# fudan-zvg/NeRF-LiDAR

Hardware: AMD Instinct MI355X
Metric: LiDAR rays/sec @128 samples/ray, 8x256 MLP; depth L1 vs reference (higher is better)
Workload: dtype f32 (sampling, hash grid) + split-bf16 x3 MFMA (density/semantic/intensity) + bf16 MFMA (view MLP); 1 GPU; C2: nuScenes 32-beam sweep, 32x1024 rays per sweep, samples (64,64,128), 8x256 NerfMLP + semantic + intensity heads, full-size fp32 hash tables; azimuth_columns_total=1024, parallelism=azimuth-sector x1, hip_graph_replay=False, weights=seeded synthetic (white-noise tables, x1500 density gain), sweep_origins=moving: step i renders sweep i mod 64 (pre-uploaded ray batches), gather_bytes_per_ray=1347584

## Files before the change

include/nerflidar_hip.h:

```cpp
#ifndef NERFLIDAR_HIP_H
#define NERFLIDAR_HIP_H

#include <stddef.h>
#include <stdint.h>

#ifdef __cplusplus
extern "C" {
#endif

#define NLR_MAX_LEVELS 4
#define NLR_MAX_GRID_LEVELS 16
#define NLR_MAX_VIEW_DEPTH 16

enum {
    NLR_OK = 0,
    NLR_ERR_INVALID = -1,
    NLR_ERR_UNSUPPORTED = -2,
    NLR_ERR_HIP = -3,
    NLR_ERR_WORKSPACE = -4
};

enum {
    NLR_PREC_F32 = 0,
    NLR_PREC_MIXED = 1,
// ... 60 lines not shown
    NlrLinear sem0, sem2;
    uint32_t use_intensity;
    NlrLinear int0, int2;
    float density_bias, rgb_premultiplier, rgb_bias, rgb_padding;
    uint32_t re_weights;
} NlrMlpDesc;

typedef struct NlrModelDesc {
    uint32_t num_levels;
    uint32_t num_samples[NLR_MAX_LEVELS];
    const NlrMlpDesc *mlps[NLR_MAX_LEVELS];
    float dilation_multiplier, dilation_bias;
    float anneal_slope, resample_padding;
    float power_lambda, std_scale;
    float bg_intensity;
    uint32_t opaque_background;
    uint32_t mlp_precision;
} NlrModelDesc;

typedef struct NlrModel NlrModel;
int nlr_model_create(const NlrModelDesc *desc, NlrModel **out, void *stream);
void nlr_model_destroy(NlrModel *m);
int nlr_model_set_table(NlrModel *m, uint32_t level, const void *table_dev, int table_dtype);

typedef struct NlrRays {
    const float *origins, *directions, *viewdirs;
    const float *radii, *near, *far;
    const float *base_x, *base_y;
} NlrRays;

typedef struct NlrRenderCfg {
    float train_frac;
    uint32_t compute_extras;
    uint32_t sample_n, sample_m;
    const float *rand_jitter[NLR_MAX_LEVELS];
    const float *rand_deg[NLR_MAX_LEVELS];
    float scale_factor;
    uint32_t shuffled_rays;
} NlrRenderCfg;

typedef struct NlrLevelOut {
    float *sdist, *tdist;
    float *weights, *density;
    float *rgb;
    float *semantic;
    float *intensity;
// ... 22 lines not shown
                     const NlrOut *out, void *workspace, size_t workspace_bytes, void *stream);

const char *nlr_kernel_names(void);

const char *nlr_build_sha(void);

#define NLR_DBG_FORCE_GENERIC 0
#define NLR_DBG_MLP_WORKGROUPS 1
#define NLR_DBG_BINNED_C4 2
#define NLR_DBG_NO_XPAIR_SCATTER 3
#define NLR_DBG_SCATTER_LEVELS 4
#define NLR_DBG_NO_SCATTER_CACHE 5
#define NLR_DBG_RAY_GROUPS 6
#define NLR_DBG_LAST_ROUTE 7
#define NLR_DBG_TRAIN_ROUTE 8
#define NLR_DBG_TRAIN_TRUNK_ROW0 9
#define NLR_DBG_TRAIN_TRUNK_ROWS 10
int nlr_debug_set(uint32_t key, int value);
int nlr_debug_get(uint32_t key);
int nlr_grid_fast_path(const int32_t *offsets_host, uint32_t L, uint32_t C, float S, uint32_t H, int table_dtype, uint32_t gridtype,
                       int align_corners, uint32_t interp);
int nlr_grid_level_plan(const int32_t *offsets_host, uint32_t L, uint32_t C, float S, uint32_t H, uint32_t gridtype, int align_corners,
                        uint32_t B, uint32_t *mode, uint32_t *step, uint32_t *lds_kind);

enum { NLR_K_RESAMPLE = 0, NLR_K_PROP = 1, NLR_K_ENCODE = 2, NLR_K_DIRBIAS = 3, NLR_K_MLP = 4, NLR_K_COMPOSITE = 5, NLR_K_COUNT = 6 };
int nlr_profile_begin(NlrModel *m);
int nlr_profile_begin_kinds(NlrModel *m, uint32_t kind_mask);
int nlr_profile_end(NlrModel *m, void *stream, float *total_ms, uint32_t *launches);

int nlr_resample_level(const float *prev_sdist, const float *prev_weights, uint32_t n_prev,
                       float dilation, float anneal, float resample_padding, uint32_t num_samples,
                       const float *rand_jitter, const float *near, const float *far,
                       float power_lambda, uint32_t N, float *sdist, float *tdist, void *stream);

int nlr_mlp_level(const NlrModel *m, uint32_t level, const NlrRays *rays, const float *tdist,
                  uint32_t N, uint32_t sample_n, uint32_t sample_m, const float *rand_deg,
                  float *features , float *density, float *rgb,
                  float *semantic, float *intensity, void *workspace, size_t workspace_bytes,
                  void *stream);

int nlr_composite_level(const float *density, const float *tdist, const float *directions,
                        const float *rgb, const float *semantic, const float *intensity,
                        const float *far, const float *origins, uint32_t N, uint32_t S,
                        uint32_t class_num, int opaque_background, float bg, int compute_extras,
                        float scale_factor, float *weights, const NlrOut *out, float *level_depth,
                        void *stream);
// ... 139 lines not shown
```

nerf-lidar_amd/csrc/nlr_api.hip:

```cpp
#include <stdarg.h>

#include <vector>

#include "nlr_kernels.h"

#include <stdlib.h>
#include "nlr_objects.h"
#include "nlr_tape.h"


static thread_local char g_err[512] = "";
void nlr_set_error(const char *fmt, ...) {
    va_list ap;
    va_start(ap, fmt);
    vsnprintf(g_err, sizeof(g_err), fmt, ap);
    va_end(ap);
}
extern "C" const char *nlr_last_error(void) { return g_err; }
extern "C" int nlr_version(void) { return 100; }
extern "C" const char *nlr_kernel_names(void) {
    return "nlr_resample_kernel,nlr_prop8_kernel,nlr_encode8_kernel,nlr_direnc_kernel,nlr_mlp_kernel,nlr_composite_kernel";
}

struct Profile {
// ... 21 lines not shown

struct MlpShape {
    uint32_t W = 0, WB = 0, D = 0, HT = 0, K = 0, int_row = 0xffffffffu, deg = 0, E = 0;
    bool use_int = false;
    uint32_t prec = NLR_PREC_MIXED;
    float rgb_premul = 1.0f, rgb_bias = 0.0f, rgb_padding = 0.001f;
};
struct LevelModel : MlpShape {
    bool is_prop = false;
    GridParams gp;
    uint32_t F = 0, S = 0;
    int re_weights = 1;
    float density_bias = -1.0f;
    float *p_w1 = nullptr, *p_b1 = nullptr, *p_w2 = nullptr;
    float p_b2 = 0.0f;
    void *tape = nullptr;
    uint32_t tape_chunks = 0;
    void *tape_lidar = nullptr;
    uint32_t tape_lidar_chunks = 0;
    float *bias_all = nullptr;
    uint32_t bias_count = 0;
    float *u_det = nullptr, *u_rand = nullptr;
    float max_jitter = 0.0f;
};

struct NlrModel {
    uint32_t num_levels = 0;
    LevelModel lv[NLR_MAX_LEVELS];
    float dilation_multiplier, dilation_bias, anneal_slope, resample_padding, power_lambda, std_scale, bg;
    uint32_t opaque, prec;
    int device = 0;
    uint32_t cus = 0;
    hipStream_t up = nullptr;
    std::vector<void *> allocs;
    mutable Profile prof;
};

static int dev_upload(NlrModel *m, const void *host, size_t bytes, void **out) {
    void *p = nullptr;
    NLR_HIP(hipMalloc(&p, bytes ? bytes : 16));
    m->allocs.push_back(p);
    if (bytes) {
        NLR_HIP(hipMemcpyAsync(p, host, bytes, hipMemcpyHostToDevice, m->up));
        NLR_HIP(hipStreamSynchronize(m->up));
    }
    *out = p;
// ... 283 lines not shown
                nlr_set_error("single_mlp / NerfMLP as proposal network has no fused path (level %u)", l);
                rc = NLR_ERR_UNSUPPORTED;
            }
        }
        if (rc) {
            nlr_model_destroy(m);
            return rc;
        }
    }
    if (hipStreamSynchronize(m->up) != hipSuccess) {
        nlr_model_destroy(m);
        NLR_FAIL(NLR_ERR_HIP, "model_create: weight upload failed");
    }
    *out = m;
    return NLR_OK;
}

extern "C" void nlr_model_destroy(NlrModel *m) {
    if (!m) return;
    for (void *p : m->allocs) (void)hipFree(p);
    delete m;
}

extern "C" int nlr_model_set_table(NlrModel *m, uint32_t level, const void *table_dev, int table_dtype) {
    NLR_CHECK_ARG(m && level < m->num_levels && table_dev, "model_set_table: bad argument");
    NLR_CHECK_ARG(table_dtype == 0 || table_dtype == 1, "model_set_table: table_dtype must be 0 or 1");
    m->lv[level].gp.table = table_dev;
    m->lv[level].gp.table_dtype = table_dtype;
    return NLR_OK;
}

extern "C" int nlr_profile_begin_kinds(NlrModel *m, uint32_t kind_mask) {
    NLR_CHECK_ARG(m != nullptr, "profile_begin: NULL model");
    for (hipEvent_t e : m->prof.ev) (void)hipEventDestroy(e);
    m->prof.ev.clear();
    m->prof.kind.clear();
    m->prof.mask = kind_mask;
    m->prof.armed = true;
    return NLR_OK;
}
extern "C" int nlr_profile_begin(NlrModel *m) { return nlr_profile_begin_kinds(m, 0xffffffffu); }

extern "C" int nlr_profile_end(NlrModel *m, void *stream, float *total_ms, uint32_t *launches) {
    NLR_CHECK_ARG(m && total_ms && launches, "profile_end: NULL argument");
    m->prof.armed = false;
    NLR_HIP(hipStreamSynchronize((hipStream_t)stream));
    for (int k = 0; k < NLR_K_COUNT; ++k) {
        total_ms[k] = 0.0f;
        launches[k] = 0;
    }
    for (size_t i = 0; i < m->prof.kind.size(); ++i) {
// ... 297 lines not shown
```

nerf-lidar_amd/csrc/nlr_common.h:

```cpp
#pragma once
#include <hip/hip_runtime.h>
#include <math.h>
#include <stdint.h>
#include <stdio.h>
#include <string.h>

#include "../../include/nerflidar_hip.h"
#include "nlr_tape.h"

#define NLR_EPS 1.1920928955078125e-07f
#define NLR_WAVE 64

void nlr_set_error(const char *fmt, ...);
#define NLR_FAIL(code, ...)         \
    do {                            \
        nlr_set_error(__VA_ARGS__); \
        return (code);              \
    } while (0)
#define NLR_CHECK_ARG(cond, ...) \
    do {                         \
        if (!(cond)) NLR_FAIL(NLR_ERR_INVALID, __VA_ARGS__); \
    } while (0)
#define NLR_HIP(call)                                                                      \
    do {                                                                                   \
// ... 7 lines not shown
        if (e_ != hipSuccess)                                                              \
            NLR_FAIL(NLR_ERR_HIP, "launch of %s failed: %s", name, hipGetErrorString(e_)); \
    } while (0)
static inline int nlr_tape_check(const char *what, size_t built, size_t program) {
    char msg[256];
    if (!nlr_tape_matches(what, built, program, msg, sizeof(msg))) NLR_FAIL(NLR_ERR_UNSUPPORTED, "%s", msg);
    return NLR_OK;
}

struct GridParams {
    const void *table;
    int32_t table_dtype;
    uint32_t L, C;
    uint32_t gridtype, align_corners, interp;
    uint32_t offset[NLR_MAX_GRID_LEVELS];
    uint32_t hsize[NLR_MAX_GRID_LEVELS];
    uint32_t res[NLR_MAX_GRID_LEVELS];
    float scale[NLR_MAX_GRID_LEVELS];
    float gsize[NLR_MAX_GRID_LEVELS];
    float inv_gsize[NLR_MAX_GRID_LEVELS];
    uint32_t dense[NLR_MAX_GRID_LEVELS];
    uint32_t mode[NLR_MAX_GRID_LEVELS];
    uint32_t step[NLR_MAX_GRID_LEVELS];
};

int nlr_fill_grid_params(GridParams *gp, const void *table, int table_dtype, const int32_t *offsets_host,
                         uint32_t L, uint32_t C, float S, uint32_t H, uint32_t gridtype, int align_corners,
                         uint32_t interp);

#ifdef __HIPCC__
__device__ __forceinline__ uint32_t nlr_grid_index(uint32_t gridtype, uint32_t align_corners, uint32_t hsize,
                                                   uint32_t res, uint32_t x, uint32_t y, uint32_t z) {
    uint32_t stride = 1, index = 0;
    const uint32_t step = align_corners ? res : res + 1;
    if (stride <= hsize) { index += x * stride; stride *= step; }
    if (stride <= hsize) { index += y * stride; stride *= step; }
    if (stride <= hsize) { index += z * stride; stride *= step; }
    if (gridtype == 0 && stride > hsize) index = x ^ (y * 2654435761u) ^ (z * 805459861u);
    return index % hsize;
}

template <int MODE>
__device__ __forceinline__ void nlr_corner_idx(const GridParams &gp, uint32_t level, const uint32_t (&pg)[3], uint32_t (&idx)[8]) {
    if (MODE == 0) {
        const uint32_t s = gp.step[level];
        const uint32_t y0 = pg[1] * s, z0 = pg[2] * s * s;
        const uint32_t y1 = y0 + s, z1 = z0 + s * s;
// ... 49 lines not shown
```

nerf-lidar_amd/csrc/nlr_encode.hip:

```cpp
#include "nlr_kernels.h"

#include <stdlib.h>

#include "nlr_cast.h"
#include "nlr_grid_level.h"
#include "nlr_level_fast.h"

template <typename T, int C>
__global__ void __launch_bounds__(256) nlr_encode_kernel(CastParams cp, GridParams gp, int re_weights, float *__restrict__ feat) {
    const uint32_t m = blockIdx.x * blockDim.x + threadIdx.x;
    const uint32_t M = cp.N * cp.S;
    if (m >= M) return;
    const uint32_t level = blockIdx.y;
    const uint32_t ray = m / cp.S, k = m - ray * cp.S;
    const RayRegs rr = nlr_load_ray(cp, ray, k);
    const float gsize = gp.gsize[level];
    float acc[C];
#pragma unroll
    for (int c = 0; c < C; ++c) acc[c] = 0.0f;
    for (uint32_t j = 0; j < cp.n; ++j) {
        const Gauss g = nlr_cast_one(cp, ray, k, j, rr);
        const float werf = re_weights ? nlr_erf_weight(g.zs, gsize) : 1.0f;
        nlr_level_accum<T, C>(gp, level, g, werf, acc);
    }
// ... 258 lines not shown
                for (int c = 0; c < 4; ++c) f0[c] = a[c] * inv_n, f1[c] = a[4 + c] * inv_n;
                continue;
            }
            float *f = nlr_feat_ptr<C>(feat, piece_major, M, m, l, gp.L);
            if constexpr (C == 4) {
                const nlr_f4 q = {a[0] * inv_n, a[1] * inv_n, a[2] * inv_n, a[3] * inv_n};
                __builtin_nontemporal_store(q, (nlr_f4 *)f);
            } else {
#pragma unroll
                for (int c = 0; c < C; ++c) f[c] = a[c] * inv_n;
            }
        }
    }
}

template <typename T, int C>
__global__ void __launch_bounds__(256) nlr_encode8_kernel(CastParams cp, GridParams gp, int re_weights, float *__restrict__ feat,
                                                          int piece_major, uint32_t nblocks, uint32_t chunk) {
    for (uint32_t b = blockIdx.x; b < nblocks; b += gridDim.x)
        nlr_encode8_block<T, C>(cp, gp, re_weights, feat, piece_major, chunk ? nlr_xcd_block(b, nblocks, chunk) : b);
}

template <typename T, int C, int LMAX>
__global__ void __launch_bounds__(256) nlr_prop8_kernel(CastParams cp, GridParams gp, PropMlpParams mp, int re_weights,
                                                        float *__restrict__ density, float *__restrict__ feat_out, uint32_t nblocks, uint32_t chunk) {
    __shared__ float sw[64 * 16 + 128];
    for (uint32_t i = threadIdx.x; i < 64 * mp.F; i += 256) sw[i] = mp.w1[i];
    if (threadIdx.x < 64) {
        sw[64 * mp.F + threadIdx.x] = mp.b1[threadIdx.x];
        sw[64 * mp.F + 64 + threadIdx.x] = mp.w2[threadIdx.x];
    }
    __syncthreads();
  for (uint32_t lb = blockIdx.x; lb < nblocks; lb += gridDim.x) {
    const uint32_t gt = (chunk ? nlr_xcd_block(lb, nblocks, chunk) : lb) * 256u + threadIdx.x;
    const uint32_t j = gt & 7;
    uint32_t pray, k;
    const bool in = nlr_slot_sample(cp, gt >> 3, pray, k);
    const uint32_t ray = NLR_DBG_RAY(pray);
    const uint32_t m = ray * cp.S + k;
    const bool active = in && j < cp.n;
    const RayRegs rr = nlr_load_ray(cp, ray, k);
    const Gauss g = nlr_cast_one(cp, ray, k, active ? j : 0, rr);
    const bool valid = active && !((g.x0 < 0 || g.x0 > 1) || (g.x1 < 0 || g.x1 > 1) || (g.x2 < 0 || g.x2 > 1));
    const float inv_s8 = __frsqrt_rn(8.0f * (g.zs * g.zs));
    const float inv_n = 1.0f / (float)cp.n;
    float feat[LMAX * C];
#pragma unroll
    for (int i = 0; i < LMAX * C; ++i) feat[i] = 0.0f;
    if (valid) {
#pragma unroll
        for (int l = 0; l < LMAX; ++l) {
            if (l < (int)gp.L) {
                const float werf = re_weights ? nlr_erf_weight_fast(inv_s8, gp.inv_gsize[l]) : 1.0f;
                float a[C];
                if (gp.mode[l] == 0) nlr_level_fast<T, C, 0>(gp, l, g.x0, g.x1, g.x2, werf, a);
                else nlr_level_fast<T, C, 1>(gp, l, g.x0, g.x1, g.x2, werf, a);
#pragma unroll
                for (int c = 0; c < C; ++c) feat[l * C + c] = a[c];
            }
        }
    }
    static_assert((LMAX * C) % 4 == 0, "feature count of the proposal kernel must be a multiple of 4");
#pragma unroll
    for (int i = 0; i < LMAX * C; i += 4) {
        float q[4] = {feat[i], feat[i + 1], feat[i + 2], feat[i + 3]};
        nlr_group8_sum_n(q);
#pragma unroll
        for (int u = 0; u < 4; ++u) feat[i + u] = q[u] * inv_n;
    }
    if (feat_out && in && j == 0)
        for (uint32_t i = 0; i < mp.F; ++i) feat_out[(size_t)m * mp.F + i] = feat[i];
    float part = 0.0f;
#pragma unroll
    for (int hh = 0; hh < 8; ++hh) {
        const uint32_t hu = hh * 8 + j;
        float a = sw[64 * mp.F + hu];
#pragma unroll
        for (int i = 0; i < LMAX * C; ++i)
            if (i < (int)mp.F) a = fmaf(sw[hu * mp.F + i], feat[i], a);
// ... 257 lines not shown
```

nerf-lidar_amd/csrc/nlr_grid.hip:

```cpp
#include "nlr_common.h"
#include "nlr_grid_level.h"

#include <hip/hip_fp16.h>

void nlr_level_scale(uint32_t L, float S, uint32_t H, float *scale, uint32_t *resolution) {
    for (uint32_t l = 0; l < L; ++l) {
        float sc = exp2f((float)l * S) * (float)H - 1.0f;
        scale[l] = sc;
        resolution[l] = (uint32_t)ceilf(sc) + 1u;
    }
}

int nlr_fill_grid_params(GridParams *gp, const void *table, int table_dtype, const int32_t *offsets_host,
                         uint32_t L, uint32_t C, float S, uint32_t H, uint32_t gridtype, int align_corners,
                         uint32_t interp) {
    NLR_CHECK_ARG(L >= 1 && L <= NLR_MAX_GRID_LEVELS, "grid: num_levels %u outside [1,%d]", L, NLR_MAX_GRID_LEVELS);
    NLR_CHECK_ARG(C == 1 || C == 2 || C == 4 || C == 8, "GridEncoding: C must be 1, 2, 4, or 8 (got %u)", C);
    NLR_CHECK_ARG(table_dtype == 0 || table_dtype == 1, "grid: table_dtype must be 0 (f32) or 1 (f16)");
    NLR_CHECK_ARG(offsets_host != nullptr, "grid: offsets (host) is NULL");
    memset(gp, 0, sizeof(*gp));
    gp->table = table;
    gp->table_dtype = table_dtype;
    gp->L = L;
    gp->C = C;
// ... 4 lines not shown
    for (uint32_t l = 0; l < L; ++l) {
        NLR_CHECK_ARG(offsets_host[l + 1] > offsets_host[l], "grid: offsets must be increasing (level %u)", l);
        gp->offset[l] = (uint32_t)offsets_host[l];
        gp->hsize[l] = (uint32_t)(offsets_host[l + 1] - offsets_host[l]);
        double r = ceil((double)H * exp2((double)l * (double)S));
        gp->gsize[l] = (float)((int)r + (align_corners ? 0 : 1));
        gp->inv_gsize[l] = 1.0f / gp->gsize[l];
        uint64_t step = align_corners ? gp->res[l] : gp->res[l] + 1, stride = 1;
        int dense = 1;
        for (int d = 0; d < 3; ++d) {
            if (stride > gp->hsize[l]) break;
            stride *= step;
        }
        if (gridtype == 0 && stride > gp->hsize[l]) dense = 0;
        gp->dense[l] = dense;
        gp->step[l] = (uint32_t)step;
        const uint32_t hs = gp->hsize[l];
        const bool all3 = (step <= hs) && (step * step <= hs);
        const bool walk = all3 && step * step * step <= hs;
        const uint64_t cmax = (uint64_t)floorf(fmaf(1.0f, gp->scale[l], align_corners ? 0.0f : 0.5f)) + 1u;
        if (walk && cmax * (1 + step + step * step) < hs) gp->mode[l] = 0;
        else if (!walk && gridtype == 0 && (hs & (hs - 1)) == 0) gp->mode[l] = 1;
        else gp->mode[l] = 2;
    }
    return NLR_OK;
}

template <typename T>
__device__ __forceinline__ float ld(const T *p);
template <>
__device__ __forceinline__ float ld<float>(const float *p) { return *p; }
template <>
__device__ __forceinline__ float ld<__half>(const __half *p) { return __half2float(*p); }

template <typename T, int C, bool DYDX>
__global__ void __launch_bounds__(256) nlr_grid_fwd_kernel(const float *__restrict__ x, GridParams gp, float *__restrict__ out,
                                                           float *__restrict__ dy_dx, uint32_t B, int out_layout) {
    const uint32_t b = blockIdx.x * blockDim.x + threadIdx.x;
    if (b >= B) return;
    const uint32_t level = blockIdx.y;
    const uint32_t L = gp.L;
    const T *grid = (const T *)gp.table + (size_t)gp.offset[level] * C;
    float *o = out_layout == 0 ? out + ((size_t)level * B + b) * C : out + (size_t)b * L * C + level * C;
    float *dd = DYDX ? dy_dx + (size_t)b * 3 * L * C + (size_t)level * 3 * C : nullptr;

    const float x0 = x[(size_t)b * 3 + 0], x1 = x[(size_t)b * 3 + 1], x2 = x[(size_t)b * 3 + 2];
// ... 711 lines not shown
```

nerf-lidar_amd/csrc/nlr_kernels.h:

```cpp
#pragma once
#include "nlr_common.h"

#define NLR_MAX_MULTI 16

struct CastParams {
    const float *origins, *directions, *base_x, *base_y, *radii;
    const float *tdist;
    const float *rand_deg;
    uint32_t N, S, n;
    uint32_t ray_groups, vote_min;
    const uint32_t *votes;
    float std_scale;
    float cosd[NLR_MAX_MULTI], sind[NLR_MAX_MULTI];
    float degj[NLR_MAX_MULTI];
};

struct PropMlpParams {
    const float *w1, *b1;
    const float *w2;
    float b2, density_bias;
    uint32_t F;
};

struct CompositeParams {
// ... 39 lines not shown
    uint32_t lidar;
};

struct DirEncParams {
    const float *viewdirs;
    const float *dirs;
    uint32_t N, deg, E;
    float *out;
    float *dnorm;
};
int nlr_launch_dnorm(const float *dirs, uint32_t N, float *dnorm, hipStream_t st);

int nlr_launch_resample(const float *prev_sdist, const float *prev_weights, uint32_t n_prev, float dilation, float anneal,
                        float pad, uint32_t S, const float *u_dev, const float *jitter, float max_jitter, const float *near,
                        const float *far, float lam, uint32_t N, float *sdist, float *tdist, hipStream_t st);
int nlr_fill_cast_params(CastParams *cp, const NlrRays *rays, const float *tdist, const float *rand_deg, uint32_t N,
                         uint32_t S, uint32_t n, uint32_t mloops, float std_scale);
int nlr_encode_features_args(CastParams *cp, GridParams *gp, const NlrRays *rays, const float *tdist, uint32_t N, uint32_t S, uint32_t sample_n,
                             uint32_t sample_m, float std_scale, const float *rand_deg, const NlrGridDesc *grid);
int nlr_launch_encode(const CastParams &cp, const GridParams &gp, int re_weights, float *feat, int piece_major, hipStream_t st);
int nlr_launch_ray_vote(const float *tdist, uint32_t N, uint32_t S, uint32_t *votes, hipStream_t st);
int nlr_launch_prop(const CastParams &cp, const GridParams &gp, const float *w1, const float *b1, const float *w2, float b2,
                    float density_bias, int re_weights, float *density, float *feat_out, hipStream_t st);
int nlr_launch_direnc(const DirEncParams &P, hipStream_t st);
int nlr_launch_mlp(const MlpParams &P, uint32_t W, uint32_t WB, uint32_t HT, uint32_t prec, uint32_t cus, hipStream_t st);
bool nlr_mlp_can_composite(uint32_t W, uint32_t WB, uint32_t HT, uint32_t prec, uint32_t F, uint32_t S, uint32_t K, bool use_int, uint64_t M,
                           uint32_t mode = 1);
int nlr_launch_composite(const CompositeParams &P, hipStream_t st);
int nlr_composite_segments(const float *density, const float *tdist, const float *directions, const float *seg, uint32_t class_num,
                           int has_intensity, const float *far, const float *origins, uint32_t N, uint32_t S, int opaque_background,
                           float bg, int compute_extras, float scale_factor, float *weights, const NlrOut *out, float *level_depth,
                           hipStream_t st, bool no_rgb = false);
int nlr_composite_level_impl(const float *density, const float *tdist, const float *directions, const float *rgb, const float *semantic,
                             const float *intensity, const float *far, const float *origins, uint32_t N, uint32_t S, uint32_t class_num,
                             int opaque_background, float bg, int compute_extras, float scale_factor, float *weights, const NlrOut *out,
                             float *level_depth, hipStream_t st, bool no_rgb);
```

nerf-lidar_amd/csrc/nlr_level_fast.h:

```cpp
#pragma once
#include "nlr_grid_level.h"

typedef float nlr_f2 __attribute__((ext_vector_type(2)));
#ifdef NLR_DBG_ENV
__device__ int nlr_dbg[8] = {0, 99, 0, 0, 0, 0, 0, 0};
#endif

template <typename T, int C>
struct NlrEntry;
template <>
struct NlrEntry<float, 1> {
    static constexpr int E = 2;
    static __device__ __forceinline__ void ld(const char *base, uint32_t off, float (&v)[1]) { v[0] = *(const float *)(base + off); }
};
template <>
struct NlrEntry<float, 2> {
    static constexpr int E = 3;
    static __device__ __forceinline__ void ld(const char *base, uint32_t off, float (&v)[2]) {
        const float2 t = *(const float2 *)(base + off);
        v[0] = t.x, v[1] = t.y;
    }
};
typedef float nlr_f4 __attribute__((ext_vector_type(4)));
template <>
// ... 100 lines not shown
template <>
struct NlrPair<__half, 4> {
    static constexpr bool ok = true;
    static __device__ __forceinline__ void ld(const char *base, uint32_t off, float (&a)[4], float (&b)[4]) {
        const nlr_uint4_a8 t = *(const nlr_uint4_a8 *)(base + off);
        const uint32_t w[4] = {t.x, t.y, t.z, t.w};
#pragma unroll
        for (int i = 0; i < 2; ++i) {
            const __half2 p = __builtin_bit_cast(__half2, w[i]), q = __builtin_bit_cast(__half2, w[2 + i]);
            a[2 * i] = __low2float(p), a[2 * i + 1] = __high2float(p), b[2 * i] = __low2float(q), b[2 * i + 1] = __high2float(q);
        }
    }
};

static inline bool nlr_level_fast_ok(const GridParams &gp) {
    if (gp.interp != 0 || gp.align_corners != 0) return false;
    const uint64_t entry = (uint64_t)gp.C * (gp.table_dtype == 0 ? 4 : 2);
    for (uint32_t l = 0; l < gp.L; ++l) {
        if (gp.mode[l] > 1) return false;
        if ((uint64_t)gp.hsize[l] * entry > (1ull << 32)) return false;
        if (gp.res[l] >= (1u << 30)) return false;
    }
    return true;
}

typedef uint32_t nlr_u2 __attribute__((ext_vector_type(2)));
typedef uint32_t nlr_u4 __attribute__((ext_vector_type(4)));
typedef uint32_t nlr_u8 __attribute__((ext_vector_type(8)));
template <int DW>
struct NlrSLoad8;
#define NLR_SLOAD8(DW, VT, OP)                                                                                                        \
    template <>                                                                                                                       \
    struct NlrSLoad8<DW> {                                                                                                            \
        typedef VT vt;                                                                                                                \
        static __device__ __forceinline__ void ld(const char *base, const uint32_t (&o)[8], VT (&q)[8]) {                             \
            asm volatile(OP " %0, %8, %9\n" OP " %1, %8, %10\n" OP " %2, %8, %11\n" OP " %3, %8, %12\n" OP " %4, %8, %13\n"      \
                         OP " %5, %8, %14\n" OP " %6, %8, %15\n" OP " %7, %8, %16\ns_waitcnt lgkmcnt(0)"                            \
                         : "=&s"(q[0]), "=&s"(q[1]), "=&s"(q[2]), "=&s"(q[3]), "=&s"(q[4]), "=&s"(q[5]), "=&s"(q[6]), "=&s"(q[7])      \
                         : "s"(base), "s"(o[0]), "s"(o[1]), "s"(o[2]), "s"(o[3]), "s"(o[4]), "s"(o[5]), "s"(o[6]), "s"(o[7])           \
                         : "memory");                                                                                                 \
        }                                                                                                                             \
    };
NLR_SLOAD8(1, uint32_t, "s_load_dword")
NLR_SLOAD8(2, nlr_u2, "s_load_dwordx2")
NLR_SLOAD8(4, nlr_u4, "s_load_dwordx4")
NLR_SLOAD8(8, nlr_u8, "s_load_dwordx8")
#undef NLR_SLOAD8
template <int DW>
__device__ __forceinline__ uint32_t nlr_dw(const typename NlrSLoad8<DW>::vt &q, int i) {
    if constexpr (DW == 1) return q;
    else return q[i];
}
template <typename T, int DW>
__device__ __forceinline__ float nlr_entry_ch(const typename NlrSLoad8<DW>::vt &q, int c) {
    if constexpr (sizeof(T) == 4) return __builtin_bit_cast(float, nlr_dw<DW>(q, c));
    else {
        const __half2 h = __builtin_bit_cast(__half2, nlr_dw<DW>(q, c >> 1));
        return (c & 1) ? __high2float(h) : __low2float(h);
    }
}

__device__ __forceinline__ uint32_t nlr_add_su(uint32_t v, uint32_t s) {
    uint32_t r;
    asm("v_add_u32 %0, %1, %2" : "=v"(r) : "s"(s), "v"(v));
    return r;
}

template <typename T, int C, int MODE>
__device__ __forceinline__ void nlr_level_fast(const GridParams &gp, uint32_t level, float x0, float x1, float x2, float werf, float (&a)[C]) {
    constexpr int E = NlrEntry<T, C>::E;
    constexpr int DW = (1 << E) / 4;
    const float scale = gp.scale[level];
    const char *base = (const char *)gp.table + ((size_t)gp.offset[level] << E);
    const float p0 = fmaf(x0, scale, 0.5f), p1 = fmaf(x1, scale, 0.5f), p2 = fmaf(x2, scale, 0.5f);
    const uint32_t g0 = (uint32_t)p0, g1 = (uint32_t)p1, g2 = (uint32_t)p2;
    const float f0 = __builtin_amdgcn_fractf(p0), f1 = __builtin_amdgcn_fractf(p1), f2 = __builtin_amdgcn_fractf(p2);
    const nlr_f2 wx = {1.0f - f0, f0};
    const float wy0 = 1.0f - f1, wz0 = 1.0f - f2;
    const nlr_f2 wxy0 = wx * wy0, wxy1 = wx * f1;
    const nlr_f2 w2[4] = {wxy0 * wz0, wxy1 * wz0, wxy0 * f2, wxy1 * f2};
    float r[C];
#pragma unroll
    for (int c = 0; c < C; ++c) r[c] = 0.0f;
    const uint32_t step = gp.step[level], sy = step << E, sz = (step * step) << E;
    const uint32_t hm = gp.hsize[level] - 1u, pa = 2654435761u & hm, pb = 805459861u & hm;
    const uint32_t mask = hm << E;
    bool uniform = false;
    uint32_t u0 = 0, u1 = 0, u2 = 0;
    if constexpr (DW >= 1) {
        u0 = __builtin_amdgcn_readfirstlane(g0), u1 = __builtin_amdgcn_readfirstlane(g1), u2 = __builtin_amdgcn_readfirstlane(g2);
        uniform = __builtin_amdgcn_ballot_w64((g0 != u0) | (g1 != u1) | (g2 != u2)) == 0ull;
#ifdef NLR_DBG_ENV
        if (nlr_dbg[3]) uniform = false;
#endif
    }
    if (uniform) {
        if constexpr (DW >= 1) {
            uint32_t so[8];
            if (MODE == 0) {
                const uint32_t ox = u0 << E, oy = u1 * sy, oz = u2 * sz;
#pragma unroll
                for (int c8 = 0; c8 < 8; ++c8) so[c8] = (ox + ((c8 & 1) << E)) + (oy + ((c8 & 2) ? sy : 0u)) + (oz + ((c8 & 4) ? sz : 0u));
            } else {
                const uint32_t hx = u0 << E, hy = (u1 << E) * pa, hz = (u2 << E) * pb;
#pragma unroll
                for (int c8 = 0; c8 < 8; ++c8)
// ... 36 lines not shown
                    for (int c8 = 0; c8 < 8; ++c8) NlrEntry<T, C>::ld_nt(base, off[c8], v[c8]);
                } else {
#pragma unroll
                    for (int c8 = 0; c8 < 8; ++c8) NlrEntry<T, C>::ld(base, off[c8], v[c8]);
                }
            } else
#endif
            {
#pragma unroll
                for (int c8 = 0; c8 < 8; ++c8) NlrEntry<T, C>::ld(base, off[c8], v[c8]);
            }
        }
#pragma unroll
        for (int c8 = 0; c8 < 8; ++c8) {
            const float w = (c8 & 1) ? w2[c8 >> 1].y : w2[c8 >> 1].x;
#pragma unroll
            for (int c = 0; c < C; ++c) r[c] = fmaf(w, v[c8][c], r[c]);
        }
    }
#pragma unroll
    for (int c = 0; c < C; ++c) a[c] = r[c] * werf;
}

#define NLR_DPP_ADD(R, CTRL) "v_add_f32_dpp " R ", " R ", " R " " CTRL " row_mask:0xf bank_mask:0xf\n"
#define NLR_Q1 "quad_perm:[1,0,3,2]"
#define NLR_Q2 "quad_perm:[2,3,0,1]"
#define NLR_HM "row_half_mirror"
__device__ __forceinline__ void nlr_group8_sum_n(float (&a)[1]) {
    asm volatile("s_nop 1\n" NLR_DPP_ADD("%0", NLR_Q1) "s_nop 1\n" NLR_DPP_ADD("%0", NLR_Q2) "s_nop 1\n" NLR_DPP_ADD("%0", NLR_HM) : "+v"(a[0]));
}
__device__ __forceinline__ void nlr_group8_sum_n(float (&a)[2]) {
    asm volatile("s_nop 1\n" NLR_DPP_ADD("%0", NLR_Q1) NLR_DPP_ADD("%1", NLR_Q1) "s_nop 0\n" NLR_DPP_ADD("%0", NLR_Q2) NLR_DPP_ADD("%1", NLR_Q2)
                 "s_nop 0\n" NLR_DPP_ADD("%0", NLR_HM) NLR_DPP_ADD("%1", NLR_HM)
                 : "+v"(a[0]), "+v"(a[1]));
}
__device__ __forceinline__ void nlr_group8_sum_n(float (&a)[4]) {
    asm volatile("s_nop 1\n" NLR_DPP_ADD("%0", NLR_Q1) NLR_DPP_ADD("%1", NLR_Q1) NLR_DPP_ADD("%2", NLR_Q1) NLR_DPP_ADD("%3", NLR_Q1)
                 NLR_DPP_ADD("%0", NLR_Q2) NLR_DPP_ADD("%1", NLR_Q2) NLR_DPP_ADD("%2", NLR_Q2) NLR_DPP_ADD("%3", NLR_Q2)
                 NLR_DPP_ADD("%0", NLR_HM) NLR_DPP_ADD("%1", NLR_HM) NLR_DPP_ADD("%2", NLR_HM) NLR_DPP_ADD("%3", NLR_HM)
                 : "+v"(a[0]), "+v"(a[1]), "+v"(a[2]), "+v"(a[3]));
}
#define NLR_DPP_ADD3(D, R, CTRL) "v_add_f32_dpp " D ", " R ", " R " " CTRL " row_mask:0xf bank_mask:0xf\n"
__device__ __forceinline__ void nlr_group8_sum_to(const float (&r)[4], float (&t)[4]) {
    asm volatile("s_nop 1\n" NLR_DPP_ADD3("%0", "%4", NLR_Q1) NLR_DPP_ADD3("%1", "%5", NLR_Q1) NLR_DPP_ADD3("%2", "%6", NLR_Q1) NLR_DPP_ADD3("%3", "%7", NLR_Q1)
                 NLR_DPP_ADD("%0", NLR_Q2) NLR_DPP_ADD("%1", NLR_Q2) NLR_DPP_ADD("%2", NLR_Q2) NLR_DPP_ADD("%3", NLR_Q2)
                 NLR_DPP_ADD("%0", NLR_HM) NLR_DPP_ADD("%1", NLR_HM) NLR_DPP_ADD("%2", NLR_HM) NLR_DPP_ADD("%3", NLR_HM)
// ... 17 lines not shown
```

nerf-lidar_amd/nerflidar_hip/models.py:

```python
from __future__ import annotations

import ctypes as C
from typing import Dict, List, Optional

import numpy as np
import torch

from . import _lib
from .config import MLPConfig, ModelConfig
from .weights import grid_layout, mlp_names, mlp_param_shapes

_RAY_KEYS = _lib.RAY_KEYS


def _f32c(a) -> np.ndarray:
    return np.ascontiguousarray(np.asarray(a, dtype=np.float32))


class Model:

    def __init__(self, mc: ModelConfig, state_dict: Dict[str, object], device="cuda:0",
                 precision: int = _lib.PREC_FAST, table_dtype=torch.float32):
        if mc.config.instance_obj:
            raise NotImplementedError("instance_obj=True (dynamic-object branch, ZI/models.py:306-315,401-477) "
                                      "is outside the fused path (SURVEY section 8f-1)")
        if mc.raydist_fn != "power_transformation":
            raise NotImplementedError("only raydist_fn='power_transformation' (the gin value) is supported")
        self.mc = mc
        self.config = mc.config
        self.device = torch.device(device)
        self.precision = precision
        self.training = False
        self.shuffled_rays = False
        self.num_levels = mc.num_levels
        self.tables: Dict[str, torch.Tensor] = {}
        self._keep = []
        self._handle = C.c_void_p(None)
        self._ws: Optional[torch.Tensor] = None
        sd = {k: (v.detach().cpu().numpy() if isinstance(v, torch.Tensor) else np.asarray(v)) for k, v in state_dict.items()}
        desc = _lib.NlrModelDesc()
        desc.num_levels = mc.num_levels
        samples = mc.level_samples()
        mlp_descs = []
        for li, (prefix, cfg) in enumerate(mlp_names(mc)):
            desc.num_samples[li] = samples[li]
            md = self._mlp_desc(prefix, cfg, sd, table_dtype)
            mlp_descs.append(md)
            desc.mlps[li] = C.pointer(md)
        desc.dilation_multiplier = mc.dilation_multiplier
        desc.dilation_bias = mc.dilation_bias
        desc.anneal_slope = mc.anneal_slope
        desc.resample_padding = mc.resample_padding
        desc.power_lambda = mc.power_lambda
        desc.std_scale = mc.std_scale
        lo, hi = mc.bg_intensity_range
        desc.bg_intensity = lo if lo == hi else (lo + hi) / 2
        desc.opaque_background = int(mc.opaque_background)
        desc.mlp_precision = precision
        _lib.call("nlr_model_create", desc, self._handle, device=self.device)
        self._keep.clear()

    def _linear(self, sd, name) -> _lib.NlrLinear:
        w, b = _f32c(sd[name + ".weight"]), _f32c(sd[name + ".bias"])
        self._keep += [w, b]
        l = _lib.NlrLinear()
        l.weight = w.ctypes.data
        l.bias = b.ctypes.data
        l.out_features, l.in_features = w.shape
        return l

    def _mlp_desc(self, prefix: str, cfg: MLPConfig, sd, table_dtype) -> _lib.NlrMlpDesc:
        md = _lib.NlrMlpDesc()
        offsets, _, pls = grid_layout(cfg)
        emb = sd[f"{prefix}.encoder.embeddings"]
        if emb.shape != (int(offsets[-1]), cfg.grid_level_dim):
            raise RuntimeError(f"{prefix}.encoder.embeddings has shape {emb.shape}, expected "
                               f"{(int(offsets[-1]), cfg.grid_level_dim)}")
        table = torch.from_numpy(_f32c(emb)).to(self.device, table_dtype).contiguous()
        self.tables[prefix] = table
        off = np.ascontiguousarray(offsets, np.int32)
        self._keep.append(off)
        g = md.grid
        g.table = table.data_ptr()
# ... 302 lines not shown
```

Baseline: 5.339 million rays/s.

## Bake proposal hash grids into dense per-cell corner bundles

At model creation, the proposal-level hash grid tables are re-laid out on device so each cell stores its eight corner entries contiguously (bundle), or stored unhashed as a dense grid when bundles exceed the budget. The proposal encoder then does one wide load per sample, or a scalar load when the whole wavefront falls in one cell, in place of eight scattered hashed gathers. The prop kernel also gets occupancy hints in its launch bounds. The cost is extra device memory (up to roughly 150 MB per grid) and a one-time bake that must be redone whenever a table is replaced.

Measured after the change: 5.405 million rays/s (median of 6 runs). 1.2% higher.

```diff
diff --git a/include/nerflidar_hip.h b/include/nerflidar_hip.h
--- a/include/nerflidar_hip.h
+++ b/include/nerflidar_hip.h
@@ -106,6 +106,12 @@
 int nlr_model_create(const NlrModelDesc *desc, NlrModel **out, void *stream);
 void nlr_model_destroy(NlrModel *m);
 int nlr_model_set_table(NlrModel *m, uint32_t level, const void *table_dev, int table_dtype);
+#define NLR_BAKE_NONE 0
+#define NLR_BAKE_BUNDLE 1
+#define NLR_BAKE_UNHASHED 2
+#define NLR_BAKE_DEFAULT_BUDGET 150994944
+int nlr_model_bake_grids(NlrModel *m, size_t budget_bytes_per_grid, void *stream);
+int nlr_model_baked(const NlrModel *m, uint32_t level, uint32_t *layout_host, uint32_t *bytes_host);
 
 typedef struct NlrRays {
     const float *origins, *directions, *viewdirs;
@@ -174,6 +180,8 @@
                        int align_corners, uint32_t interp);
 int nlr_grid_level_plan(const int32_t *offsets_host, uint32_t L, uint32_t C, float S, uint32_t H, uint32_t gridtype, int align_corners,
                         uint32_t B, uint32_t *mode, uint32_t *step, uint32_t *lds_kind);
+int nlr_grid_bake_plan(const NlrGridDesc *grid, size_t budget_bytes, uint32_t *layout_host, uint32_t *cells_host, uint32_t *off32_host,
+                       uint32_t *bytes_host, uint32_t *total32_host);
 
 enum { NLR_K_RESAMPLE = 0, NLR_K_PROP = 1, NLR_K_ENCODE = 2, NLR_K_DIRBIAS = 3, NLR_K_MLP = 4, NLR_K_COMPOSITE = 5, NLR_K_COUNT = 6 };
 int nlr_profile_begin(NlrModel *m);
diff --git a/nerf-lidar_amd/csrc/nlr_api.hip b/nerf-lidar_amd/csrc/nlr_api.hip
--- a/nerf-lidar_amd/csrc/nlr_api.hip
+++ b/nerf-lidar_amd/csrc/nlr_api.hip
@@ -67,6 +67,8 @@
     uint32_t bias_count = 0;
     float *u_det = nullptr, *u_rand = nullptr;
     float max_jitter = 0.0f;
+    void *baked = nullptr;
+    uint64_t baked_bytes[NLR_MAX_GRID_LEVELS] = {};
 };
 
 struct NlrModel {
@@ -396,11 +398,59 @@
     delete m;
 }
 
+static void drop_baked(NlrModel *m, LevelModel &lv) {
+    lv.gp.baked = nullptr;
+    lv.gp.bake_mask = 0;
+    for (uint32_t g = 0; g < NLR_MAX_GRID_LEVELS; ++g) lv.gp.level_off[g] = lv.gp.offset[g], lv.baked_bytes[g] = 0;
+    if (!lv.baked) return;
+    for (size_t i = 0; i < m->allocs.size(); ++i)
+        if (m->allocs[i] == lv.baked) {
+            m->allocs.erase(m->allocs.begin() + i);
+            break;
+        }
+    (void)hipFree(lv.baked);
+    lv.baked = nullptr;
+}
+
 extern "C" int nlr_model_set_table(NlrModel *m, uint32_t level, const void *table_dev, int table_dtype) {
     NLR_CHECK_ARG(m && level < m->num_levels && table_dev, "model_set_table: bad argument");
     NLR_CHECK_ARG(table_dtype == 0 || table_dtype == 1, "model_set_table: table_dtype must be 0 or 1");
+    drop_baked(m, m->lv[level]);
     m->lv[level].gp.table = table_dev;
     m->lv[level].gp.table_dtype = table_dtype;
+    return NLR_OK;
+}
+
+#define NLR_BAKE_MODEL_CAP (1ull << 30)
+
+extern "C" int nlr_model_bake_grids(NlrModel *m, size_t budget_bytes_per_grid, void *stream) {
+    NLR_CHECK_ARG(m != nullptr, "model_bake_grids: NULL model");
+    uint32_t nprop = 0;
+    for (uint32_t l = 0; l < m->num_levels; ++l) nprop += m->lv[l].is_prop ? 1u : 0u;
+    if (!nprop) return NLR_OK;
+    const uint64_t cap = (NLR_BAKE_MODEL_CAP - 1) / nprop;
+    const uint64_t budget = budget_bytes_per_grid < cap ? budget_bytes_per_grid : cap;
+    hipStream_t st = (hipStream_t)stream;
+    for (uint32_t l = 0; l < m->num_levels; ++l) {
+        LevelModel &lv = m->lv[l];
+        if (!lv.is_prop) continue;
+        drop_baked(m, lv);
+        if (!budget) continue;
+        const int rc = nlr_bake_grid(&lv.gp, budget, &lv.baked, lv.baked_bytes, st);
+        if (rc) return rc;
+        if (lv.baked) m->allocs.push_back(lv.baked);
+    }
+    NLR_HIP(hipStreamSynchronize(st));
+    return NLR_OK;
+}
+
+extern "C" int nlr_model_baked(const NlrModel *m, uint32_t level, uint32_t *layout_host, uint32_t *bytes_host) {
+    NLR_CHECK_ARG(m && level < m->num_levels && layout_host && bytes_host, "model_baked: bad argument");
+    const LevelModel &lv = m->lv[level];
+    for (uint32_t g = 0; g < lv.gp.L; ++g) {
+        layout_host[g] = nlr_bake_layout(lv.gp, g);
+        bytes_host[g] = (uint32_t)lv.baked_bytes[g];
+    }
     return NLR_OK;
 }
 
diff --git a/nerf-lidar_amd/csrc/nlr_bake.hip b/nerf-lidar_amd/csrc/nlr_bake.hip
--- /dev/null
+++ b/nerf-lidar_amd/csrc/nlr_bake.hip
@@ -0,0 +1,112 @@
+#include "nlr_kernels.h"
+#undef NLR_DBG_ENV
+#include "nlr_level_fast.h"
+
+#include <type_traits>
+
+template <int EB>
+__device__ __forceinline__ void nlr_bake_copy(const char *__restrict__ src, uint32_t si, bool ok, char *__restrict__ dst, size_t di) {
+    using W = typename std::conditional<(EB >= 4), uint32_t, uint16_t>::type;
+    constexpr int NW = EB / (int)sizeof(W);
+    const W *s = (const W *)(src + (size_t)si * EB);
+    W *d = (W *)(dst + di * EB);
+#pragma unroll
+    for (int k = 0; k < NW; ++k) d[k] = ok ? s[k] : (W)0;
+}
+
+template <int EB, int MODE>
+__global__ void __launch_bounds__(256) nlr_bake_bundle_kernel(GridParams gp, uint32_t level, uint32_t n, char *__restrict__ out) {
+    const uint32_t cell = blockIdx.x * 256u + threadIdx.x;
+    if (cell >= n * n * n) return;
+    const uint32_t pg[3] = {cell % n, (cell / n) % n, cell / (n * n)};
+    uint32_t idx[8];
+    nlr_corner_idx<MODE>(gp, level, pg, idx);
+    const char *src = (const char *)gp.table + (size_t)gp.offset[level] * EB;
+    const uint32_t hsize = gp.hsize[level];
+#pragma unroll
+    for (int c8 = 0; c8 < 8; ++c8) nlr_bake_copy<EB>(src, idx[c8], idx[c8] < hsize, out, (size_t)cell * 8 + c8);
+}
+
+template <int EB>
+__global__ void __launch_bounds__(256) nlr_bake_unhash_kernel(GridParams gp, uint32_t level, uint32_t count, char *__restrict__ out) {
+    const uint32_t i = blockIdx.x * 256u + threadIdx.x;
+    if (i >= count) return;
+    const uint32_t s = gp.step[level];
+    const uint32_t pg[3] = {i % s, (i / s) % s, i / (s * s)};
+    uint32_t idx[8];
+    nlr_corner_idx<1>(gp, level, pg, idx);
+    nlr_bake_copy<EB>((const char *)gp.table + (size_t)gp.offset[level] * EB, idx[0], true, out, i);
+}
+
+template <int EB>
+static void nlr_bake_level(const GridParams &gp, const NlrBakePlan &plan, uint32_t l, char *out, hipStream_t st) {
+    if (plan.layout[l] == NLR_BAKE_BUNDLE) {
+        const uint32_t n = plan.cells[l];
+        const dim3 grid((n * n * n + 255u) / 256u);
+        if (gp.mode[l] == 0) hipLaunchKernelGGL((nlr_bake_bundle_kernel<EB, 0>), grid, dim3(256), 0, st, gp, l, n, out);
+        else hipLaunchKernelGGL((nlr_bake_bundle_kernel<EB, 1>), grid, dim3(256), 0, st, gp, l, n, out);
+    } else {
+        const uint32_t count = (uint32_t)(plan.bytes[l] / EB);
+        hipLaunchKernelGGL((nlr_bake_unhash_kernel<EB>), dim3((count + 255u) / 256u), dim3(256), 0, st, gp, l, count, out);
+    }
+}
+
+int nlr_bake_grid(GridParams *gp, uint64_t budget, void **alloc, uint64_t *bytes, hipStream_t st) {
+    NlrBakePlan plan;
+    nlr_bake_plan(*gp, budget, &plan);
+    *alloc = nullptr;
+    gp->baked = nullptr;
+    gp->bake_mask = 0;
+    for (uint32_t l = 0; l < NLR_MAX_GRID_LEVELS; ++l) gp->level_off[l] = gp->offset[l], bytes[l] = 0;
+    if (!plan.total) return NLR_OK;
+    NLR_CHECK_ARG(gp->table != nullptr, "bake: the level has no table");
+    NLR_CHECK_ARG((plan.total >> 5) < (1ull << 32), "bake: %llu bytes do not fit the 32-bit level offsets", (unsigned long long)plan.total);
+    void *p = nullptr;
+    NLR_HIP(hipMalloc(&p, plan.total));
+    const uint32_t EB = gp->C * (gp->table_dtype == 0 ? 4u : 2u);
+    for (uint32_t l = 0; l < gp->L; ++l) {
+        if (plan.layout[l] == NLR_BAKE_NONE) continue;
+        char *out = (char *)p + plan.offset[l];
+        switch (EB) {
+            case 2: nlr_bake_level<2>(*gp, plan, l, out, st); break;
+            case 4: nlr_bake_level<4>(*gp, plan, l, out, st); break;
+            case 8: nlr_bake_level<8>(*gp, plan, l, out, st); break;
+            case 16: nlr_bake_level<16>(*gp, plan, l, out, st); break;
+            default: nlr_bake_level<32>(*gp, plan, l, out, st); break;
+        }
+        const hipError_t e = hipGetLastError();
+        if (e != hipSuccess) {
+            (void)hipFree(p);
+            NLR_FAIL(NLR_ERR_HIP, "launch of nlr_bake kernel failed: %s", hipGetErrorString(e));
+        }
+    }
+    for (uint32_t l = 0; l < gp->L; ++l) {
+        if (plan.layout[l] == NLR_BAKE_BUNDLE) gp->bake_mask |= 1u << l;
+        if (plan.layout[l] == NLR_BAKE_UNHASHED) gp->bake_mask |= 1u << (16 + l);
+        if (plan.layout[l] != NLR_BAKE_NONE) gp->level_off[l] = (uint32_t)(plan.offset[l] >> 5);
+        bytes[l] = plan.bytes[l];
+    }
+    gp->baked = p;
+    *alloc = p;
+    return NLR_OK;
+}
+
+extern "C" int nlr_grid_bake_plan(const NlrGridDesc *grid, size_t budget_bytes, uint32_t *layout_host, uint32_t *cells_host, uint32_t *off32_host,
+                                  uint32_t *bytes_host, uint32_t *total32_host) {
+    NLR_CHECK_ARG(grid && grid->offsets && layout_host && cells_host && off32_host && bytes_host && total32_host, "grid_bake_plan: NULL argument");
+    GridParams gp;
+    const int rc = nlr_fill_grid_params(&gp, grid->table, grid->table_dtype, grid->offsets, grid->num_levels, grid->level_dim,
+                                        grid->log2_per_level_scale, grid->base_resolution, grid->gridtype, (int)grid->align_corners, grid->interp);
+    if (rc) return rc;
+    NlrBakePlan plan;
+    nlr_bake_plan(gp, budget_bytes, &plan);
+    NLR_CHECK_ARG((plan.total >> 5) < (1ull << 32), "grid_bake_plan: %llu bytes do not fit the 32-bit level offsets", (unsigned long long)plan.total);
+    for (uint32_t l = 0; l < gp.L; ++l) {
+        layout_host[l] = plan.layout[l];
+        cells_host[l] = plan.cells[l];
+        off32_host[l] = (uint32_t)(plan.offset[l] >> 5);
+        bytes_host[l] = (uint32_t)plan.bytes[l];
+    }
+    *total32_host = (uint32_t)(plan.total >> 5);
+    return NLR_OK;
+}
diff --git a/nerf-lidar_amd/csrc/nlr_common.h b/nerf-lidar_amd/csrc/nlr_common.h
--- a/nerf-lidar_amd/csrc/nlr_common.h
+++ b/nerf-lidar_amd/csrc/nlr_common.h
@@ -53,7 +53,15 @@
     uint32_t dense[NLR_MAX_GRID_LEVELS];
     uint32_t mode[NLR_MAX_GRID_LEVELS];
     uint32_t step[NLR_MAX_GRID_LEVELS];
+    const void *baked;
+    uint32_t bake_mask;
+    uint32_t hashed_mask;
+    uint32_t level_off[NLR_MAX_GRID_LEVELS];
 };
+static_assert(NLR_MAX_GRID_LEVELS <= 16, "GridParams.bake_mask holds two bits per level");
+__host__ __device__ static inline uint32_t nlr_bake_layout(const GridParams &gp, uint32_t l) {
+    return ((gp.bake_mask >> l) & 1u) | ((gp.bake_mask >> (15u + l)) & 2u);
+}
 
 int nlr_fill_grid_params(GridParams *gp, const void *table, int table_dtype, const int32_t *offsets_host,
                          uint32_t L, uint32_t C, float S, uint32_t H, uint32_t gridtype, int align_corners,
diff --git a/nerf-lidar_amd/csrc/nlr_encode.hip b/nerf-lidar_amd/csrc/nlr_encode.hip
--- a/nerf-lidar_amd/csrc/nlr_encode.hip
+++ b/nerf-lidar_amd/csrc/nlr_encode.hip
@@ -304,7 +304,11 @@
 }
 
 template <typename T, int C, int LMAX>
-__global__ void __launch_bounds__(256) nlr_prop8_kernel(CastParams cp, GridParams gp, PropMlpParams mp, int re_weights,
+constexpr int nlr_prop8_waves() {
+    return C == 1 && LMAX == 8 ? 7 : (C == 1 && sizeof(T) == 4 ? 6 : 5);
+}
+template <typename T, int C, int LMAX>
+__global__ void __launch_bounds__(256, (nlr_prop8_waves<T, C, LMAX>())) nlr_prop8_kernel(CastParams cp, GridParams gp, PropMlpParams mp, int re_weights,
                                                         float *__restrict__ density, float *__restrict__ feat_out, uint32_t nblocks, uint32_t chunk) {
     __shared__ float sw[64 * 16 + 128];
     for (uint32_t i = threadIdx.x; i < 64 * mp.F; i += 256) sw[i] = mp.w1[i];
@@ -335,8 +339,7 @@
             if (l < (int)gp.L) {
                 const float werf = re_weights ? nlr_erf_weight_fast(inv_s8, gp.inv_gsize[l]) : 1.0f;
                 float a[C];
-                if (gp.mode[l] == 0) nlr_level_fast<T, C, 0>(gp, l, g.x0, g.x1, g.x2, werf, a);
-                else nlr_level_fast<T, C, 1>(gp, l, g.x0, g.x1, g.x2, werf, a);
+                nlr_level_fast_baked<T, C>(gp, l, g.x0, g.x1, g.x2, werf, a);
 #pragma unroll
                 for (int c = 0; c < C; ++c) feat[l * C + c] = a[c];
             }
diff --git a/nerf-lidar_amd/csrc/nlr_grid.hip b/nerf-lidar_amd/csrc/nlr_grid.hip
--- a/nerf-lidar_amd/csrc/nlr_grid.hip
+++ b/nerf-lidar_amd/csrc/nlr_grid.hip
@@ -50,6 +50,8 @@
         if (walk && cmax * (1 + step + step * step) < hs) gp->mode[l] = 0;
         else if (!walk && gridtype == 0 && (hs & (hs - 1)) == 0) gp->mode[l] = 1;
         else gp->mode[l] = 2;
+        if (gp->mode[l] == 1) gp->hashed_mask |= 1u << l;
+        gp->level_off[l] = gp->offset[l];
     }
     return NLR_OK;
 }
diff --git a/nerf-lidar_amd/csrc/nlr_kernels.h b/nerf-lidar_amd/csrc/nlr_kernels.h
--- a/nerf-lidar_amd/csrc/nlr_kernels.h
+++ b/nerf-lidar_amd/csrc/nlr_kernels.h
@@ -85,6 +85,7 @@
 int nlr_launch_ray_vote(const float *tdist, uint32_t N, uint32_t S, uint32_t *votes, hipStream_t st);
 int nlr_launch_prop(const CastParams &cp, const GridParams &gp, const float *w1, const float *b1, const float *w2, float b2,
                     float density_bias, int re_weights, float *density, float *feat_out, hipStream_t st);
+int nlr_bake_grid(GridParams *gp, uint64_t budget, void **alloc, uint64_t *bytes, hipStream_t st);
 int nlr_launch_direnc(const DirEncParams &P, hipStream_t st);
 int nlr_launch_mlp(const MlpParams &P, uint32_t W, uint32_t WB, uint32_t HT, uint32_t prec, uint32_t cus, hipStream_t st);
 bool nlr_mlp_can_composite(uint32_t W, uint32_t WB, uint32_t HT, uint32_t prec, uint32_t F, uint32_t S, uint32_t K, bool use_int, uint64_t M,
diff --git a/nerf-lidar_amd/csrc/nlr_level_fast.h b/nerf-lidar_amd/csrc/nlr_level_fast.h
--- a/nerf-lidar_amd/csrc/nlr_level_fast.h
+++ b/nerf-lidar_amd/csrc/nlr_level_fast.h
@@ -146,6 +146,39 @@
         if (gp.res[l] >= (1u << 30)) return false;
     }
     return true;
+}
+
+struct NlrBakePlan {
+    uint32_t layout[NLR_MAX_GRID_LEVELS];
+    uint32_t cells[NLR_MAX_GRID_LEVELS];
+    uint64_t offset[NLR_MAX_GRID_LEVELS];
+    uint64_t bytes[NLR_MAX_GRID_LEVELS];
+    uint64_t total;
+};
+static inline void nlr_bake_plan(const GridParams &gp, uint64_t budget, NlrBakePlan *p) {
+    memset(p, 0, sizeof(*p));
+    const bool fast = nlr_level_fast_ok(gp);
+    const uint64_t entry = (uint64_t)gp.C * (gp.table_dtype == 0 ? 4 : 2);
+    uint64_t used = 0;
+    for (uint32_t l = 0; l < gp.L && l < NLR_MAX_GRID_LEVELS; ++l) {
+        const uint64_t step = gp.step[l];
+        p->cells[l] = (uint32_t)(step - 1);
+        if (!fast || gp.mode[l] > 1 || step < 2) continue;
+        if ((uint64_t)floorf(fmaf(1.0f, gp.scale[l], 0.5f)) > step - 2) continue;
+        const uint64_t n = step - 1;
+        const uint64_t cap = 1ull << 32;
+        const uint64_t bundle = (n * n < cap && 8 * entry <= 32) ? n * n * n * 8 * entry : cap;
+        const uint64_t dense = (step * step < cap) ? step * step * step * entry : cap;
+        const uint64_t left = budget > used ? budget - used : 0;
+        uint64_t bytes = 0;
+        if (bundle < cap && bundle <= left) p->layout[l] = NLR_BAKE_BUNDLE, bytes = bundle;
+        else if (gp.mode[l] == 1 && dense < cap && ((dense + 31) & ~31ull) <= left) p->layout[l] = NLR_BAKE_UNHASHED, bytes = dense;
+        else continue;
+        p->offset[l] = used;
+        p->bytes[l] = bytes;
+        used += (bytes + 31) & ~31ull;
+    }
+    p->total = used;
 }
 
 typedef uint32_t nlr_u2 __attribute__((ext_vector_type(2)));
@@ -190,12 +223,48 @@
     return r;
 }
 
-template <typename T, int C, int MODE>
-__device__ __forceinline__ void nlr_level_fast(const GridParams &gp, uint32_t level, float x0, float x1, float x2, float werf, float (&a)[C]) {
+template <int RDW>
+struct NlrSLoad1;
+template <>
+struct NlrSLoad1<4> {
+    typedef nlr_u4 vt;
+    static __device__ __forceinline__ void ld(const char *base, uint32_t off, vt &q) {
+        asm volatile("s_load_dwordx4 %0, %1, %2\ns_waitcnt lgkmcnt(0)" : "=&s"(q) : "s"(base), "s"(off) : "memory");
+    }
+};
+template <>
+struct NlrSLoad1<8> {
+    typedef nlr_u8 vt;
+    static __device__ __forceinline__ void ld(const char *base, uint32_t off, vt &q) {
+        asm volatile("s_load_dwordx8 %0, %1, %2\ns_waitcnt lgkmcnt(0)" : "=&s"(q) : "s"(base), "s"(off) : "memory");
+    }
+};
+template <typename T, int C, typename DW>
+__device__ __forceinline__ void nlr_bundle_fma(DW &&dw, const nlr_f2 (&w2)[4], float (&r)[C]) {
+#pragma unroll
+    for (int c8 = 0; c8 < 8; ++c8) {
+        const float w = (c8 & 1) ? w2[c8 >> 1].y : w2[c8 >> 1].x;
+#pragma unroll
+        for (int c = 0; c < C; ++c) {
+            const int e = c8 * C + c;
+            float v;
+            if constexpr (sizeof(T) == 4) v = __builtin_bit_cast(float, dw(e));
+            else {
+                const uint32_t d = dw(e >> 1);
+                const __half2 h = __builtin_bit_cast(__half2, d);
+                v = (e & 1) ? __high2float(h) : __low2float(h);
+            }
+            r[c] = fmaf(w, v, r[c]);
+        }
+    }
+}
+
+template <typename T, int C, int MODE, bool BUNDLE = false>
+__device__ __forceinline__ void nlr_level_fast_at(const GridParams &gp, uint32_t level, const char *base, float x0, float x1, float x2, float werf,
+                                                  float (&a)[C]) {
     constexpr int E = NlrEntry<T, C>::E;
     constexpr int DW = (1 << E) / 4;
     const float scale = gp.scale[level];
-    const char *base = (const char *)gp.table + ((size_t)gp.offset[level] << E);
     const float p0 = fmaf(x0, scale, 0.5f), p1 = fmaf(x1, scale, 0.5f), p2 = fmaf(x2, scale, 0.5f);
     const uint32_t g0 = (uint32_t)p0, g1 = (uint32_t)p1, g2 = (uint32_t)p2;
     const float f0 = __builtin_amdgcn_fractf(p0), f1 = __builtin_amdgcn_fractf(p1), f2 = __builtin_amdgcn_fractf(p2);
@@ -206,6 +275,34 @@
     float r[C];
 #pragma unroll
     for (int c = 0; c < C; ++c) r[c] = 0.0f;
+    if constexpr (BUNDLE) {
+        constexpr int K = E + 3, RDW = (1 << K) / 4;
+        static_assert(RDW == 4 || RDW == 8, "cell bundles are records of 16 or 32 bytes");
+        const uint32_t n = gp.step[level] - 1u, ny = n << K, nz = (n * n) << K;
+        const uint32_t u0 = __builtin_amdgcn_readfirstlane(g0), u1 = __builtin_amdgcn_readfirstlane(g1), u2 = __builtin_amdgcn_readfirstlane(g2);
+        bool uniform = __builtin_amdgcn_ballot_w64((g0 != u0) | (g1 != u1) | (g2 != u2)) == 0ull;
+#ifdef NLR_DBG_ENV
+        if (nlr_dbg[3]) uniform = false;
+#endif
+        if (uniform) {
+            typename NlrSLoad1<RDW>::vt q;
+            NlrSLoad1<RDW>::ld(base, (u0 << K) + u1 * ny + u2 * nz, q);
+            nlr_bundle_fma<T, C>([&](int i) -> uint32_t { return q[i]; }, w2, r);
+        } else {
+            const uint32_t off = (g0 << K) + g1 * ny + g2 * nz;
+            uint32_t d[RDW];
+            const nlr_u4 t = *(const nlr_u4 *)(base + off);
+            d[0] = t.x, d[1] = t.y, d[2] = t.z, d[3] = t.w;
+            if constexpr (RDW == 8) {
+                const nlr_u4 u = *(const nlr_u4 *)(base + off + 16);
+                d[4] = u.x, d[5] = u.y, d[6] = u.z, d[7] = u.w;
+            }
+            nlr_bundle_fma<T, C>([&](int i) -> uint32_t { return d[i]; }, w2, r);
+        }
+#pragma unroll
+        for (int c = 0; c < C; ++c) a[c] = r[c] * werf;
+        return;
+    }
     const uint32_t step = gp.step[level], sy = step << E, sz = (step * step) << E;
     const uint32_t hm = gp.hsize[level] - 1u, pa = 2654435761u & hm, pb = 805459861u & hm;
     const uint32_t mask = hm << E;
@@ -288,6 +385,28 @@
     for (int c = 0; c < C; ++c) a[c] = r[c] * werf;
 }
 
+template <typename T, int C, int MODE>
+__device__ __forceinline__ void nlr_level_fast(const GridParams &gp, uint32_t level, float x0, float x1, float x2, float werf, float (&a)[C]) {
+    const char *base = (const char *)gp.table + ((size_t)gp.offset[level] << NlrEntry<T, C>::E);
+    nlr_level_fast_at<T, C, MODE>(gp, level, base, x0, x1, x2, werf, a);
+}
+
+template <typename T, int C>
+__device__ __forceinline__ void nlr_level_fast_baked(const GridParams &gp, uint32_t level, float x0, float x1, float x2, float werf, float (&a)[C]) {
+    constexpr int E = NlrEntry<T, C>::E;
+    const uint32_t bake = nlr_bake_layout(gp, level);
+    const size_t off = gp.level_off[level];
+    const char *base = (bake ? (const char *)gp.baked : (const char *)gp.table) + (off << (bake ? 5 : E));
+    if constexpr (8 * C * sizeof(T) <= 32) {
+        if (bake == NLR_BAKE_BUNDLE) {
+            nlr_level_fast_at<T, C, 0, true>(gp, level, base, x0, x1, x2, werf, a);
+            return;
+        }
+    }
+    if (bake == NLR_BAKE_UNHASHED || !((gp.hashed_mask >> level) & 1u)) nlr_level_fast_at<T, C, 0>(gp, level, base, x0, x1, x2, werf, a);
+    else nlr_level_fast_at<T, C, 1>(gp, level, base, x0, x1, x2, werf, a);
+}
+
 #define NLR_DPP_ADD(R, CTRL) "v_add_f32_dpp " R ", " R ", " R " " CTRL " row_mask:0xf bank_mask:0xf\n"
 #define NLR_Q1 "quad_perm:[1,0,3,2]"
 #define NLR_Q2 "quad_perm:[2,3,0,1]"
diff --git a/nerf-lidar_amd/nerflidar_hip/models.py b/nerf-lidar_amd/nerflidar_hip/models.py
--- a/nerf-lidar_amd/nerflidar_hip/models.py
+++ b/nerf-lidar_amd/nerflidar_hip/models.py
@@ -20,7 +20,8 @@
 class Model:
 
     def __init__(self, mc: ModelConfig, state_dict: Dict[str, object], device="cuda:0",
-                 precision: int = _lib.PREC_FAST, table_dtype=torch.float32):
+                 precision: int = _lib.PREC_FAST, table_dtype=torch.float32,
+                 bake_grids: Optional[int] = _lib.DEFINES["NLR_BAKE_DEFAULT_BUDGET"]):
         if mc.config.instance_obj:
             raise NotImplementedError("instance_obj=True (dynamic-object branch, ZI/models.py:306-315,401-477) "
                                       "is outside the fused path (SURVEY section 8f-1)")
@@ -59,6 +60,16 @@
         desc.mlp_precision = precision
         _lib.call("nlr_model_create", desc, self._handle, device=self.device)
         self._keep.clear()
+        self.bake_grids(bake_grids)
+
+    def bake_grids(self, budget: Optional[int] = _lib.DEFINES["NLR_BAKE_DEFAULT_BUDGET"]) -> None:
+        _lib.call("nlr_model_bake_grids", self._handle, int(budget or 0), device=self.device)
+
+    def baked(self, level: int):
+        lay, nb = (np.zeros(_lib.NLR_MAX_GRID_LEVELS, np.uint32) for _ in range(2))
+        _lib.check(_lib.lib().nlr_model_baked(self._handle, level, lay.ctypes.data, nb.ctypes.data), "nlr_model_baked")
+        L = mlp_names(self.mc)[level][1].grid_num_levels
+        return lay[:L].tolist(), nb[:L].tolist()
 
     def _linear(self, sd, name) -> _lib.NlrLinear:
         w, b = _f32c(sd[name + ".weight"]), _f32c(sd[name + ".bias"])
```
